# nikkolasg/playsnark

Measured on NVIDIA B200. Metric: g1_msm_points_per_s, higher is better.
Workload: dtype u32

## Files before the change

### playsnark_b200/build.py

```python
from __future__ import annotations

import glob
import os
import re
import subprocess
import sys
from concurrent.futures import ThreadPoolExecutor

HERE = os.path.dirname(os.path.abspath(__file__))
ROOT = os.path.dirname(HERE)
CSRC = os.path.join(HERE, "csrc")
OBJ = os.path.join(HERE, "_build")
LIB = os.path.join(HERE, "libplaysnark_b200.so")

CU_SOURCES = [os.path.join(CSRC, f) for f in ("capi.cu", "capi_poly.cu", "capi_multi.cu", "capi_verify.cu", "group_g1.cu", "group_g2.cu", "accum_g2.cu")
              if os.path.exists(os.path.join(CSRC, f))]

NVCC_FLAGS = [
    "-gencode", "arch=compute_100a,code=sm_100a", "-O3", "-std=c++17", "--expt-relaxed-constexpr",
    "-lineinfo", "-Xcompiler", "-fPIC",
]

_INC = re.compile(r'^\s*#\s*include\s+"([^"]+)"', re.M)


def _deps(path: str, seen=None):
    seen = set() if seen is None else seen
    path = os.path.normpath(path)
    if path in seen or not os.path.exists(path):
        return seen
    seen.add(path)
    with open(path) as f:
        for inc in _INC.findall(f.read()):
            _deps(os.path.join(os.path.dirname(path), inc), seen)
    return seen


def _sources():
    return sorted(glob.glob(os.path.join(CSRC, "*.cu")) + glob.glob(os.path.join(CSRC, "*.cuh")) +
                  [os.path.join(ROOT, "include", "playsnark_b200.h")])


def stale(target: str, sources) -> bool:
    if not os.path.exists(target):
        return True
    t = os.path.getmtime(target)
    return any(os.path.getmtime(s) > t for s in sources)


def build_cuda(force: bool = False, verbose: bool = False, out: str = LIB, extra_flags=()) -> str:
    if not force and not extra_flags and not stale(out, _sources()):
        return out
    nvcc = os.environ.get("NVCC", "nvcc")
    obj_dir = OBJ if out == LIB else out + ".obj"
    os.makedirs(obj_dir, exist_ok=True)
    jobs = []
    for src in CU_SOURCES:
        obj = os.path.join(obj_dir, os.path.basename(src)[:-3] + ".o")
        if force or extra_flags or stale(obj, _deps(src)):
            jobs.append((src, obj))
    threads = max(1, (os.cpu_count() or 2) // max(1, len(jobs)))

    def compile_one(job):
        src, obj = job
        cmd = [nvcc] + NVCC_FLAGS + list(extra_flags) + (["-Xptxas", "-v"] if verbose else []) + \
              ["-split-compile", str(threads), "-c", "-o", obj, src]
        print("[playsnark_b200] " + " ".join(cmd), file=sys.stderr)
        subprocess.check_call(cmd, cwd=ROOT)

    if jobs:
        with ThreadPoolExecutor(max_workers=len(jobs)) as ex:
            list(ex.map(compile_one, jobs))
    objs = [os.path.join(obj_dir, os.path.basename(s)[:-3] + ".o") for s in CU_SOURCES]
    cmd = [nvcc, "-gencode", "arch=compute_100a,code=sm_100a", "-shared", "-o", out] + objs
    print("[playsnark_b200] " + " ".join(cmd), file=sys.stderr)
    subprocess.check_call(cmd, cwd=ROOT)
    return out


def build_variant(name: str, flags, tus=("capi_poly.cu",)) -> str:
    build_cuda()
    nvcc = os.environ.get("NVCC", "nvcc")
    vdir = os.path.join(OBJ, "variants")
    os.makedirs(vdir, exist_ok=True)
    objs = []
    for src in CU_SOURCES:
        base = os.path.basename(src)
        if base in tus:
            obj = os.path.join(vdir, "%s_%s.o" % (base[:-3], name))
            if stale(obj, _deps(src)):
                cmd = [nvcc] + NVCC_FLAGS + list(flags) + ["-split-compile", "0", "-c", "-o", obj, src]
                print("[playsnark_b200] " + " ".join(cmd), file=sys.stderr)
                subprocess.check_call(cmd, cwd=ROOT)
        else:
            obj = os.path.join(OBJ, base[:-3] + ".o")
        objs.append(obj)
    os.makedirs(os.path.join(HERE, "variants"), exist_ok=True)
    out = os.path.join(HERE, "variants", "lib_%s.so" % name)
    subprocess.check_call([nvcc, "-gencode", "arch=compute_100a,code=sm_100a", "-shared", "-o", out] + objs, cwd=ROOT)
    return out


TEST_BUILD = os.path.join(ROOT, "tests", "_build")
DEVICE_HARNESS = os.path.join(ROOT, "tests", "device_arith.cu")


def can_write(dir_path: str) -> bool:
    while not os.path.isdir(dir_path):
        parent = os.path.dirname(dir_path)
        if parent == dir_path:
            return False
        dir_path = parent
    return os.access(dir_path, os.W_OK | os.X_OK)


def build_device_harness(out_dir: str = TEST_BUILD) -> str:
    so = os.path.join(out_dir, "libdevice_arith.so")
    if not stale(so, _deps(DEVICE_HARNESS)):
        return so
    os.makedirs(out_dir, exist_ok=True)
    tmp = "%s.%d.tmp" % (so, os.getpid())
    nvcc = os.environ.get("NVCC", "nvcc")
    cmd = [nvcc] + NVCC_FLAGS + ["-split-compile", "0", "-shared", "-o", tmp, DEVICE_HARNESS]
    print("[playsnark_b200] " + " ".join(cmd), file=sys.stderr)
    try:
        subprocess.check_call(cmd, cwd=ROOT)
        os.replace(tmp, so)
    finally:
        if os.path.exists(tmp):
            os.remove(tmp)
    return so


def build_host_emulation(out_dir: str) -> str:
    os.makedirs(out_dir, exist_ok=True)
    so = os.path.join(out_dir, "libps_hostemu.so")
    if not stale(so, _sources()):
        return so
    jobs = []
    for src in CU_SOURCES:
        obj = os.path.join(out_dir, "emu_" + os.path.basename(src)[:-3] + ".o")
        if stale(obj, _deps(src)):
            jobs.append((src, obj))

    def compile_one(job):
        src, obj = job
        subprocess.check_call(["g++", "-O2", "-std=c++17", "-x", "c++", "-DPS_HOST_EMU", "-fPIC", "-c", "-o", obj, src], cwd=ROOT)

    if jobs:
        with ThreadPoolExecutor(max_workers=len(jobs)) as ex:
            list(ex.map(compile_one, jobs))
    objs = [os.path.join(out_dir, "emu_" + os.path.basename(s)[:-3] + ".o") for s in CU_SOURCES]
    subprocess.check_call(["g++", "-shared", "-o", so] + objs + ["-lpthread"], cwd=ROOT)
    return so


if __name__ == "__main__":
    build_cuda(force="--force" in sys.argv, verbose="-v" in sys.argv)
```

### playsnark_b200/csrc/msm.cuh

```cuda
#pragma once
#include "group_ops.cuh"
#include "team.cuh"

namespace ps {

PS_DEV int msm_seg_of(const MsmPlan& p, uint32_t i) {
  int k = 0;
  while (k + 1 < p.nseg && i >= p.seg[k + 1].start) k++;
  return k;
}

PS_DEV void msm_load_scalar(const uint32_t* scalars, uint32_t i, int mont, uint32_t k[8], bool& neg) {
  Fr x;
#pragma unroll
  for (int j = 0; j < 8; j++) x.v[j] = scalars[(size_t)i * 8 + j];
  if (mont) x = x.from_mont();
  uint32_t t = ptx_sub_cc(FrParams::HALF(0), x.v[0]);
#pragma unroll
  for (int j = 1; j < 8; j++) t = ptx_subc_cc(FrParams::HALF(j), x.v[j]);
  uint32_t borrow = ptx_subc(0, 0);
  neg = borrow != 0;
  if (neg) {
    uint32_t m[8];
    m[0] = ptx_sub_cc(FrParams::MOD(0), x.v[0]);
#pragma unroll
    for (int j = 1; j < 8; j++) m[j] = ptx_subc_cc(FrParams::MOD(j), x.v[j]);
#pragma unroll
    for (int j = 0; j < 8; j++) x.v[j] = m[j];
  }
#pragma unroll
  for (int j = 0; j < 8; j++) k[j] = x.v[j];
}

PS_DEV uint32_t msm_take_bits(uint32_t k[8], int c) {
  uint32_t v = k[0] & ((1u << c) - 1);
#pragma unroll
  for (int j = 0; j < 7; j++) k[j] = (k[j] >> c) | (k[j + 1] << (32 - c));
  k[7] >>= c;
  return v;
}

PS_DEV bool msm_next_digit(uint32_t k[8], int c, uint32_t& carry, uint32_t& mag, bool& dneg) {
  uint32_t v = msm_take_bits(k, c) + carry;
  uint32_t half = 1u << (c - 1);
  if (v > half) { mag = (1u << c) - v; dneg = true; carry = 1; }
  else { mag = v; dneg = false; carry = 0; }
  return mag != 0;
}

struct MsmCountK {
  static constexpr int BLOCK = 256;
  PS_DEV static void run(uint32_t i, MsmPlan p, uint32_t* count, uint32_t* ranks) {
    const MsmSeg sg = p.seg[msm_seg_of(p, i)];
    uint32_t k[8]; bool neg;
    msm_load_scalar(sg.scalars, i - sg.start, (int)sg.mont, k, neg);
    uint32_t carry = 0;
    const uint32_t b0 = sg.set * (uint32_t)p.S * p.D;
    for (int w = 0; w < p.W; w++) {
      uint32_t mag; bool dneg;
      uint32_t rank = 0xFFFFFFFFu;
      if (msm_next_digit(k, p.c, carry, mag, dneg)) {
        uint32_t b = b0 + (uint32_t)(w / p.T) * p.D + (mag - 1);
        rank = ps_atomic_add(count + b, 1u);
      }
      ranks[(size_t)w * p.total + i] = rank;
    }
  }
};

struct MsmScatterK {
  static constexpr int BLOCK = 256;
  PS_DEV static void run(uint32_t i, MsmPlan p, const uint32_t* off, const uint32_t* ranks, uint32_t* ent) {
    const MsmSeg sg = p.seg[msm_seg_of(p, i)];
    uint32_t k[8]; bool neg;
    msm_load_scalar(sg.scalars, i - sg.start, (int)sg.mont, k, neg);
    uint32_t carry = 0;
    const uint32_t b0 = sg.set * (uint32_t)p.S * p.D, nbase = p.nbase[sg.set], pt = p.toff[sg.set] + sg.first + (i - sg.start);
    for (int w = 0; w < p.W; w++) {
      uint32_t mag; bool dneg;
      if (msm_next_digit(k, p.c, carry, mag, dneg)) {
        uint32_t b = b0 + (uint32_t)(w / p.T) * p.D + (mag - 1);
        uint32_t pos = off[b] + ranks[(size_t)w * p.total + i];
        uint32_t idx = (uint32_t)(w % p.T) * nbase + pt;
        ent[pos] = idx | ((neg != dneg) ? 0x80000000u : 0u);
      }
    }
  }
};

PS_DEV uint32_t msm_find_bucket(const uint32_t* off, uint32_t nb, uint32_t pos) {
  uint32_t lo = 0, hi = nb;
  while (hi - lo > 1) {
    uint32_t mid = lo + (hi - lo) / 2;
    if (off[mid] <= pos) lo = mid; else hi = mid;
  }
  return lo;
}

template <class F>
PS_DEV Affine<F> msm_load_point(const Affine<F>* tab, uint32_t e) {
  Affine<F> p = tab[e & 0x7FFFFFFFu];
  if (e >> 31) p.y = p.y.neg();
  return p;
}

#ifndef PS_G1_MINB
#define PS_G1_MINB 3
#endif
#ifndef PS_G2_MINB
#define PS_G2_MINB 2
#endif
#ifndef PS_ACC_BLOCK
#define PS_ACC_BLOCK 128
#endif
template <class F>
struct MsmAccumK {
  static constexpr int BLOCK = PS_ACC_BLOCK;
  static constexpr int MIN_BLOCKS = sizeof(F) == sizeof(Fp) ? PS_G1_MINB : PS_G2_MINB;
  using Self = MsmAccumK<F>;
  PS_DEV static void run(uint32_t tid, uint32_t nb, uint32_t L, const Affine<F>* tab, const uint32_t* ent,
                         const uint32_t* off, XYZZ<F>* buckets, XYZZ<F>* slot_pt, int32_t* slot_bid,
                         uint8_t* slot_fl) {
    const uint32_t M = off[nb];
    const uint32_t head = 2 * tid, tail = 2 * tid + 1;
    slot_bid[head] = -1; slot_bid[tail] = -1;
    uint64_t p0 = (uint64_t)tid * L;
    if (p0 >= M) return;
    uint32_t cur = (uint32_t)p0;
    uint32_t end = (M - cur > L) ? cur + L : M;
    uint32_t b = msm_find_bucket(off, nb, cur);
    bool head_open = off[b] < cur;
    uint32_t bend = off[b + 1];
    XYZZ<F> acc = XYZZ<F>::inf();
    for (; cur < end; cur++) {
      if (cur == bend) {
        flush(b, acc, head_open, true, head, tail, buckets, slot_pt, slot_bid, slot_fl);
        acc = XYZZ<F>::inf();
        head_open = false;
        b++;
        while (off[b + 1] <= cur) b++;
        bend = off[b + 1];
      }
      xyzz_madd(acc, msm_load_point(tab, ent[cur]));
    }
    flush(b, acc, head_open, bend <= end, head, tail, buckets, slot_pt, slot_bid, slot_fl);
  }
  PS_DEV static void flush(uint32_t b, const XYZZ<F>& acc, bool head_open, bool closed, uint32_t head, uint32_t tail,
                           XYZZ<F>* buckets, XYZZ<F>* slot_pt, int32_t* slot_bid, uint8_t* slot_fl) {
    if (closed && !head_open) {
      buckets[b] = acc;
    } else {
      uint32_t s = head_open ? head : tail;
      slot_pt[s] = acc;
      slot_bid[s] = (int32_t)b;
      slot_fl[s] = (uint8_t)((head_open ? 1 : 0) | (closed ? 0 : 2));
    }
  }
};

template <bool T> struct Coop;
template <> struct Coop<false> {
  static constexpr uint32_t LANES = 1;
  PS_DEV explicit Coop(uint32_t&) {}
  template <class F> PS_DEV void add(XYZZ<F>& acc, const XYZZ<F>& q) const { xyzz_add_c(acc, q); }
  template <class F> PS_DEV void dbl(XYZZ<F>& p) const { p = xyzz_dbl_c(p); }
  PS_DEV bool writer() const { return true; }
  PS_DEV bool idle() const { return false; }
  PS_DEV void sync() const {}
};
template <> struct Coop<true> {
  static constexpr uint32_t LANES = TEAM;
  TeamCtx tc;
  PS_DEV explicit Coop(uint32_t& tid) : tc(TeamCtx::of(tid)) { tid >>= 2; }
  template <class F> PS_DEV void add(XYZZ<F>& acc, const XYZZ<F>& q) const { xyzz_add_t(acc, q, tc); }
  template <class F> PS_DEV void dbl(XYZZ<F>& p) const { xyzz_dbl_t(p, tc); }
  PS_DEV bool writer() const { return tc.tl == 0; }
  PS_DEV bool idle() const {
#ifdef __CUDA_ARCH__
    return false;
#else
    return tc.tl != 0;
#endif
  }
  PS_DEV void sync() const { tc.sync(); }
};

template <class F, bool T>
struct MsmRunMergeK {
  static constexpr int BLOCK = 128;
  static constexpr uint32_t RUN_MAX = 32;
  PS_DEV static void run(uint32_t t, uint32_t n_chunks, XYZZ<F>* buckets, XYZZ<F>* slot_pt, int32_t* slot_bid,
                         const uint8_t* slot_fl) {
    Coop<T> co(t);
    if (co.idle()) return;
    const uint32_t a = 2 * t + 1;
    int32_t bid = slot_bid[a];
    if (bid < 0 || slot_fl[a] != 2) return;
    uint32_t len = 0;
    for (uint32_t j = 1; j <= RUN_MAX && t + j < n_chunks; j++) {
      uint32_t h = 2 * (t + j);
      if (slot_bid[h] != bid) return;
      if (slot_fl[h] == 1) { len = j; break; }
    }
    if (!len) return;
    XYZZ<F> acc = slot_pt[a];
    for (uint32_t j = 1; j <= len; j++) co.add(acc, slot_pt[2 * (t + j)]);
    co.sync();
    if (!co.writer()) return;
    buckets[bid] = acc;
    slot_bid[a] = -1;
    for (uint32_t j = 1; j <= len; j++) slot_bid[2 * (t + j)] = -1;
  }
};

template <class F, bool T>
struct MsmCombineK {
  static constexpr int BLOCK = 128;
  PS_DEV static void flush(int32_t bid, const XYZZ<F>& acc, bool cl, bool cr, int final_pass, uint32_t tid,
                           XYZZ<F>* buckets, XYZZ<F>* out_pt, int32_t* out_bid, uint8_t* out_fl) {
    if (bid < 0) return;
    if (final_pass || (!cl && !cr)) { buckets[bid] = acc; return; }
    uint32_t s = cl ? 2 * tid : 2 * tid + 1;
    out_pt[s] = acc; out_bid[s] = bid; out_fl[s] = (uint8_t)((cl ? 1 : 0) | (cr ? 2 : 0));
  }
  PS_DEV static void run(uint32_t tid, uint32_t n_in, uint32_t f, const XYZZ<F>* in_pt, const int32_t* in_bid,
                         const uint8_t* in_fl, XYZZ<F>* buckets, XYZZ<F>* out_pt, int32_t* out_bid,
                         uint8_t* out_fl, int final_pass) {
    Coop<T> co(tid);
    if (co.idle()) return;
    const bool wr = co.writer();
    if (wr) { out_bid[2 * tid] = -1; out_bid[2 * tid + 1] = -1; }
    int32_t cur = -1; bool cl = false, cr = false;
    XYZZ<F> acc = XYZZ<F>::inf();
    for (uint32_t i = 0; i < f; i++) {
      uint64_t j = (uint64_t)tid * f + i;
      if (j >= n_in) break;
      int32_t bid = in_bid[j];
      if (bid < 0) continue;
      uint8_t fl = in_fl[j];
      if (bid != cur) {
        if (wr) flush(cur, acc, cl, cr, final_pass, tid, buckets, out_pt, out_bid, out_fl);
        cur = bid; acc = in_pt[j]; cl = fl & 1; cr = (fl & 2) != 0;
      } else {
        co.add(acc, in_pt[j]); cr = (fl & 2) != 0;
      }
    }
    if (wr) flush(cur, acc, cl, cr, final_pass, tid, buckets, out_pt, out_bid, out_fl);
  }
};

template <class F, bool T>
struct MsmReduceFirstK {
  static constexpr int BLOCK = 128;
  PS_DEV static void run(uint32_t tid, uint32_t D, uint32_t G, uint32_t g, const XYZZ<F>* buckets, XYZZ<F>* acc_out,
                         XYZZ<F>* run_out) {
    Coop<T> co(tid);
    if (co.idle()) return;
    uint32_t s = tid / G, j = tid % G;
    const XYZZ<F>* B = buckets + (size_t)s * D + (size_t)j * g;
    XYZZ<F> rr = XYZZ<F>::inf(), ww = XYZZ<F>::inf();
    for (uint32_t i = g; i-- > 0;) {
      co.add(rr, B[i]);
      co.add(ww, rr);
    }
    if (co.writer()) { acc_out[tid] = ww; run_out[tid] = rr; }
  }
};

template <class F, bool T>
struct MsmReduceK {
  static constexpr int BLOCK = 64;
  PS_DEV static void run(uint32_t tid, uint32_t n_in, uint32_t n_out, uint32_t f, int log_len, const XYZZ<F>* acc_in,
                         const XYZZ<F>* run_in, XYZZ<F>* acc_out, XYZZ<F>* run_out) {
    Coop<T> co(tid);
    if (co.idle()) return;
    uint32_t s = tid / n_out, j = tid % n_out;
    const XYZZ<F>* A = acc_in + (size_t)s * n_in + (size_t)j * f;
    const XYZZ<F>* R = run_in + (size_t)s * n_in + (size_t)j * f;
    XYZZ<F> asum = XYZZ<F>::inf(), rr = XYZZ<F>::inf(), ww = XYZZ<F>::inf();
    for (uint32_t i = f; i-- > 0;) {
      if ((size_t)j * f + i >= n_in) continue;
      co.add(asum, A[i]);
      co.add(rr, R[i]);
      if (i > 0) co.add(ww, rr);
    }
    for (int d = 0; d < log_len; d++) co.dbl(ww);
    co.add(asum, ww);
    if (co.writer()) { acc_out[tid] = asum; run_out[tid] = rr; }
  }
};

template <class F, bool T>
struct MsmBitGatherK {
  static constexpr int BLOCK = 64;
  PS_DEV static void run(uint32_t tid, uint32_t G, int g, const XYZZ<F>* acc, const XYZZ<F>* run, XYZZ<F>* Y) {
    Coop<T> co(tid);
    if (co.idle()) return;
    const uint32_t half = G / 2;
    uint32_t s = tid / ((uint32_t)(g + 1) * half), rem = tid % ((uint32_t)(g + 1) * half);
    uint32_t r = rem / half, i = rem % half;
    XYZZ<F> y;
    if (r == 0) {
      y = acc[(size_t)s * G + 2 * i];
      co.add(y, acc[(size_t)s * G + 2 * i + 1]);
    } else {
      uint32_t k = r - 1;
      uint32_t j = ((i >> k) << (k + 1)) | (1u << k) | (i & ((1u << k) - 1));
      y = run[(size_t)s * G + j];
    }
    if (co.writer()) Y[tid] = y;
  }
};
template <class F, bool T>
struct MsmPairSumK {
  static constexpr int BLOCK = 64;
  PS_DEV static void run(uint32_t tid, uint32_t n_in, const XYZZ<F>* in, XYZZ<F>* out) {
    Coop<T> co(tid);
    if (co.idle()) return;
    uint32_t half = n_in / 2;
    uint32_t row = tid / half, i = tid % half;
    XYZZ<F> y = in[(size_t)row * n_in + 2 * i];
    co.add(y, in[(size_t)row * n_in + 2 * i + 1]);
    if (co.writer()) out[tid] = y;
  }
};
template <class F, bool T>
struct MsmBitFinalK {
  static constexpr int BLOCK = 32;
  PS_DEV static void run(uint32_t s, int g, int log_len, const XYZZ<F>* Y, XYZZ<F>* out) {
    Coop<T> co(s);
    if (co.idle()) return;
    const XYZZ<F>* row = Y + (size_t)s * (g + 1);
    XYZZ<F> r = XYZZ<F>::inf();
    for (int k = g - 1; k >= 0; k--) {
      co.dbl(r);
      co.add(r, row[k + 1]);
    }
    for (int d = 0; d < log_len; d++) co.dbl(r);
    co.add(r, row[0]);
    if (co.writer()) out[s] = r;
  }
};

template <class F, bool T>
struct MsmFinalK {
  static constexpr int BLOCK = 32;
  PS_DEV static void run(uint32_t tid, int S, int shift, const XYZZ<F>* sets, XYZZ<F>* out) {
    Coop<T> co(tid);
    if (co.idle()) return;
    XYZZ<F> r = XYZZ<F>::inf();
    for (int s = S - 1; s >= 0; s--) {
      for (int d = 0; d < shift; d++) co.dbl(r);
      co.add(r, sets[(size_t)tid * S + s]);
    }
    if (co.writer()) out[tid] = r;
  }
};

template <class F, bool T>
struct MsmSumK {
  static constexpr int BLOCK = 32;
  PS_DEV static void run(uint32_t tid, uint32_t count, const XYZZ<F>* in, XYZZ<F>* out) {
    Coop<T> co(tid);
    if (co.idle()) return;
    if (tid != 0) return;
    XYZZ<F> r = XYZZ<F>::inf();
    for (uint32_t i = 0; i < count; i++) co.add(r, in[i]);
    if (co.writer()) *out = r;
  }
};

#if PS_GPU
static constexpr int SCAN_THREADS = 256;
static constexpr int SCAN_ITEMS = 8;
static constexpr int SCAN_TILE = SCAN_THREADS * SCAN_ITEMS;

static __global__ void __launch_bounds__(SCAN_THREADS) k_scan_tiles(const uint32_t* in, uint32_t* out, uint32_t* tile_sums, uint32_t n) {
  __shared__ uint32_t warp_sums[SCAN_THREADS / 32];
  uint32_t base = blockIdx.x * SCAN_TILE + threadIdx.x * SCAN_ITEMS;
  uint32_t v[SCAN_ITEMS];
  uint32_t local = 0;
#pragma unroll
  for (int i = 0; i < SCAN_ITEMS; i++) { v[i] = (base + i < n) ? in[base + i] : 0; local += v[i]; }
  uint32_t lane = threadIdx.x & 31, wid = threadIdx.x >> 5;
  uint32_t inc = local;
#pragma unroll
  for (int d = 1; d < 32; d <<= 1) { uint32_t t = __shfl_up_sync(0xffffffffu, inc, d); if (lane >= d) inc += t; }
  if (lane == 31) warp_sums[wid] = inc;
  __syncthreads();
  if (wid == 0) {
    uint32_t ws = lane < SCAN_THREADS / 32 ? warp_sums[lane] : 0;
#pragma unroll
    for (int d = 1; d < 32; d <<= 1) { uint32_t t = __shfl_up_sync(0xffffffffu, ws, d); if (lane >= d) ws += t; }
    if (lane < SCAN_THREADS / 32) warp_sums[lane] = ws;
  }
  __syncthreads();
  uint32_t excl = inc - local + (wid ? warp_sums[wid - 1] : 0);
#pragma unroll
  for (int i = 0; i < SCAN_ITEMS; i++) { if (base + i < n) out[base + i] = excl; excl += v[i]; }
  if (threadIdx.x == SCAN_THREADS - 1) tile_sums[blockIdx.x] = warp_sums[SCAN_THREADS / 32 - 1];
}
static __global__ void __launch_bounds__(1024) k_scan_sums(uint32_t* sums, uint32_t n) {
  __shared__ uint32_t warp_sums[32];
  __shared__ uint32_t carry_s;
  if (threadIdx.x == 0) carry_s = 0;
  __syncthreads();
  uint32_t lane = threadIdx.x & 31, wid = threadIdx.x >> 5;
  for (uint32_t base = 0; base < n; base += 1024) {
    uint32_t idx = base + threadIdx.x;
    uint32_t v = idx < n ? sums[idx] : 0;
    uint32_t inc = v;
#pragma unroll
    for (int d = 1; d < 32; d <<= 1) { uint32_t t = __shfl_up_sync(0xffffffffu, inc, d); if (lane >= d) inc += t; }
    if (lane == 31) warp_sums[wid] = inc;
    __syncthreads();
    if (wid == 0) {
      uint32_t ws = warp_sums[lane];
#pragma unroll
      for (int d = 1; d < 32; d <<= 1) { uint32_t t = __shfl_up_sync(0xffffffffu, ws, d); if (lane >= d) ws += t; }
      warp_sums[lane] = ws;
    }
    __syncthreads();
    uint32_t carry = carry_s;
    uint32_t excl = carry + inc - v + (wid ? warp_sums[wid - 1] : 0);
    if (idx < n) sums[idx] = excl;
    __syncthreads();
    if (threadIdx.x == 1023) carry_s = carry + warp_sums[31];
    __syncthreads();
  }
}
static __global__ void __launch_bounds__(SCAN_THREADS) k_scan_add(uint32_t* out, const uint32_t* tile_sums, uint32_t n) {
  uint32_t base = blockIdx.x * SCAN_TILE + threadIdx.x * SCAN_ITEMS;
  uint32_t add = tile_sums[blockIdx.x];
#pragma unroll
  for (int i = 0; i < SCAN_ITEMS; i++) if (base + i < n) out[base + i] += add;
}
#endif

inline int exclusive_scan_u32(ps_stream_t st, const uint32_t* in, uint32_t* out, uint32_t* tile_sums, uint32_t n) {
#if PS_GPU
  uint32_t tiles = (n + SCAN_TILE - 1) / SCAN_TILE;
  k_scan_tiles<<<tiles, SCAN_THREADS, 0, st>>>(in, out, tile_sums, n);
  k_scan_sums<<<1, 1024, 0, st>>>(tile_sums, tiles);
  k_scan_add<<<tiles, SCAN_THREADS, 0, st>>>(out, tile_sums, n);
  PS_CUDA_TRY(cudaGetLastError());
  launch_counter() += 3;
#else
  (void)st; (void)tile_sums;
  uint32_t acc = 0;
  for (uint32_t i = 0; i < n; i++) { uint32_t v = in[i]; out[i] = acc; acc += v; }
#endif
  return PS_OK;
}

struct MsmStageScatterK {
  static constexpr int BLOCK = 256;
  PS_DEV static void run(uint32_t j, int shift, const uint32_t* part_count, const uint32_t* staging, uint32_t* ent) {
    const uint32_t part = j >> shift, k = j & ((1u << shift) - 1);
    if (k >= part_count[part]) return;
    const uint32_t pos = staging[2 * (size_t)j], val = staging[2 * (size_t)j + 1];
    ent[pos] = val;
  }
};
constexpr int SCATTER2_WMAX = 16;
#ifndef PS_SCATTER2_BLOCK
#define PS_SCATTER2_BLOCK 512
#endif
constexpr int SCATTER2_BLOCK = PS_SCATTER2_BLOCK;
#if PS_GPU
static __global__ void __launch_bounds__(SCATTER2_BLOCK) k_scatter_stage(MsmPlan p, const uint32_t* off, const uint32_t* ranks,
                                                             uint32_t* part_count, uint32_t* staging, int shift, uint32_t nparts) {
  extern __shared__ uint32_t sh_scatter[];
  uint32_t* hist = sh_scatter;
  uint32_t* base = sh_scatter + nparts;
  for (uint32_t q = threadIdx.x; q < nparts; q += blockDim.x) hist[q] = 0;
  __syncthreads();
  const uint32_t i = blockIdx.x * blockDim.x + threadIdx.x;
  uint32_t pos[SCATTER2_WMAX], val[SCATTER2_WMAX], lr[SCATTER2_WMAX];
#pragma unroll
  for (int w = 0; w < SCATTER2_WMAX; w++) pos[w] = 0xFFFFFFFFu;
  if (i < p.total) {
    const MsmSeg sg = p.seg[msm_seg_of(p, i)];
    uint32_t k[8]; bool neg;
    msm_load_scalar(sg.scalars, i - sg.start, (int)sg.mont, k, neg);
    uint32_t carry = 0;
    const uint32_t b0 = sg.set * (uint32_t)p.S * p.D, nbase = p.nbase[sg.set], pt = p.toff[sg.set] + sg.first + (i - sg.start);
#pragma unroll
    for (int w = 0; w < SCATTER2_WMAX; w++) {
      if (w < p.W) {
        uint32_t mag; bool dneg;
        if (msm_next_digit(k, p.c, carry, mag, dneg)) {
          const uint32_t b = b0 + (uint32_t)(w / p.T) * p.D + (mag - 1);
          pos[w] = off[b] + ranks[(size_t)w * p.total + i];
          val[w] = ((uint32_t)(w % p.T) * nbase + pt) | ((neg != dneg) ? 0x80000000u : 0u);
          lr[w] = atomicAdd(&hist[pos[w] >> shift], 1u);
        }
      }
    }
  }
  __syncthreads();
  for (uint32_t q = threadIdx.x; q < nparts; q += blockDim.x)
    if (hist[q]) base[q] = atomicAdd(&part_count[q], hist[q]);
  __syncthreads();
#pragma unroll
  for (int w = 0; w < SCATTER2_WMAX; w++) {
    if (pos[w] != 0xFFFFFFFFu) {
      const uint32_t part = pos[w] >> shift;
      const size_t slot = ((size_t)part << shift) + base[part] + lr[w];
      reinterpret_cast<uint2*>(staging)[slot] = make_uint2(pos[w], val[w]);
    }
  }
}
#endif
inline int scatter_stage(ps_stream_t st, const MsmPlan& p, const uint32_t* off, const uint32_t* ranks, uint32_t* part_count,
                         uint32_t* staging, int shift, uint32_t nparts) {
#if PS_GPU
  const uint32_t blocks = (p.total + SCATTER2_BLOCK - 1) / SCATTER2_BLOCK;
  k_scatter_stage<<<blocks, SCATTER2_BLOCK, 2 * nparts * sizeof(uint32_t), st>>>(p, off, ranks, part_count, staging, shift, nparts);
  PS_CUDA_TRY(cudaGetLastError());
  launch_counter()++;
#else
  (void)st; (void)nparts;
  for (uint32_t i = 0; i < p.total; i++) {
    const MsmSeg sg = p.seg[msm_seg_of(p, i)];
    uint32_t k[8]; bool neg;
    msm_load_scalar(sg.scalars, i - sg.start, (int)sg.mont, k, neg);
    uint32_t carry = 0;
    const uint32_t b0 = sg.set * (uint32_t)p.S * p.D, nbase = p.nbase[sg.set], pt = p.toff[sg.set] + sg.first + (i - sg.start);
    for (int w = 0; w < p.W; w++) {
      uint32_t mag; bool dneg;
      if (!msm_next_digit(k, p.c, carry, mag, dneg)) continue;
      const uint32_t b = b0 + (uint32_t)(w / p.T) * p.D + (mag - 1);
      const uint32_t pos = off[b] + ranks[(size_t)w * p.total + i];
      const uint32_t part = pos >> shift;
      const size_t slot = ((size_t)part << shift) + part_count[part]++;
      staging[2 * slot] = pos;
      staging[2 * slot + 1] = ((uint32_t)(w % p.T) * nbase + pt) | ((neg != dneg) ? 0x80000000u : 0u);
    }
  }
#endif
  return PS_OK;
}

template <class F>
inline int launch_accum(ps_stream_t st, size_t T1, uint32_t nb, uint32_t L, const Affine<F>* tab, const uint32_t* ent, const uint32_t* off,
                        XYZZ<F>* buckets, XYZZ<F>* slot_pt, int32_t* slot_bid, uint8_t* slot_fl) {
  PS_LAUNCH(MsmAccumK<F>, st, T1, nb, L, tab, ent, off, buckets, slot_pt, slot_bid, slot_fl);
  return PS_OK;
}
int launch_accum_g2(ps_stream_t st, size_t T1, uint32_t nb, uint32_t L, const Affine<Fp2>* tab, const uint32_t* ent, const uint32_t* off,
                    XYZZ<Fp2>* buckets, XYZZ<Fp2>* slot_pt, int32_t* slot_bid, uint8_t* slot_fl);
template <>
inline int launch_accum<Fp2>(ps_stream_t st, size_t T1, uint32_t nb, uint32_t L, const Affine<Fp2>* tab, const uint32_t* ent,
                             const uint32_t* off, XYZZ<Fp2>* buckets, XYZZ<Fp2>* slot_pt, int32_t* slot_bid, uint8_t* slot_fl) {
  return launch_accum_g2(st, T1, nb, L, tab, ent, off, buckets, slot_pt, slot_bid, slot_fl);
}

#ifndef PS_TEAM_MAX_ITEMS
#define PS_TEAM_MAX_ITEMS 65536
#endif
template <template <class, bool> class K, class F, class... Args>
inline int launch_coop(bool team, ps_stream_t st, size_t items, Args... args) {
  if (team && items <= PS_TEAM_MAX_ITEMS) return ps_launch<K<F, true>>(st, items * TEAM, args...);
  return ps_launch<K<F, false>>(st, items, args...);
}

template <class F>
int msm_run_batch(ps_ctx* ctx, const MsmPlan& g, const Affine<F>* tab, XYZZ<F>* d_out) {
  ps_stream_t st = ctx->stream;
  Arena& ar = ctx->arena;
  if (g.nsets < 1 || g.nsets > MSM_MAX_SEG || g.nseg < 0 || g.nseg > MSM_MAX_SEG) return PS_ERR_ARG;
  if (g.total == 0) return dev_memset(d_out, 0, (size_t)g.nsets * sizeof(XYZZ<F>), st);
  const int S_all = g.nsets * g.S;
  const uint32_t nb = (uint32_t)S_all * g.D;
  const size_t max_ent = (size_t)g.total * g.W;
  if (max_ent >= 0xFFFFFFFFull || (uint64_t)S_all * g.D >= 0x7FFFFFFFull) return PS_ERR_UNSUPPORTED;

  const size_t avg_bucket = max_ent / nb + 1;
  uint32_t L0 = 8;
  while (L0 < 512 && L0 < avg_bucket) L0 <<= 1;
  if (L0 < 512 && max_ent / (2 * (size_t)L0) >= 400000) L0 <<= 1;
  const size_t R = (size_t)ctx->sm_count * MsmAccumK<F>::MIN_BLOCKS * MsmAccumK<F>::BLOCK;
  size_t waves = (max_ent + R * L0 - 1) / (R * L0);
  if (ctx->msm_wave_floor && L0 <= 128 && waves > 1 && waves < 6) waves = max_ent / (R * L0);
  uint32_t L = waves >= 6 ? L0 : (uint32_t)((max_ent + waves * R - 1) / (waves * R));
  if (L < 8) L = 8;
  const size_t T1 = (max_ent + L - 1) / L;
  const uint32_t CF = 64;
  const bool team = ctx->msm_team != 0;

  uint32_t* count = ar.take<uint32_t>((size_t)nb + 1);
  uint32_t* off = ar.take<uint32_t>((size_t)nb + 1);
  uint32_t* tile_sums = ar.take<uint32_t>((size_t)nb / 2048 + 2);
  uint32_t* ranks = ar.take<uint32_t>(max_ent);
  uint32_t* ent = ar.take<uint32_t>(max_ent);
  XYZZ<F>* buckets = ar.take<XYZZ<F>>(nb);
  if (!count || !off || !tile_sums || !ranks || !ent || !buckets) return PS_ERR_ALLOC;

  ctx->ev_valid = false;
  PS_TRY(ctx_event(ctx, 0));
  PS_TRY(dev_memset(count, 0, ((size_t)nb + 1) * 4, st));
  PS_TRY(dev_memset(buckets, 0, (size_t)nb * sizeof(XYZZ<F>), st));
  PS_LAUNCH(MsmCountK, st, g.total, g, count, ranks);
  PS_TRY(exclusive_scan_u32(st, count, off, tile_sums, nb + 1));
  const bool two_pass = g.W <= SCATTER2_WMAX && (ctx->msm_scatter == 2 || (ctx->msm_scatter == 1 && max_ent >= ((size_t)1 << 27)));
  if (two_pass) {
    int shift = 20;
    while ((max_ent >> shift) >= 1024) shift++;
    const uint32_t nparts = (uint32_t)((max_ent + ((size_t)1 << shift) - 1) >> shift);
    uint32_t* part_count = ar.take<uint32_t>(nparts);
    uint32_t* staging = ar.take<uint32_t>(2 * ((size_t)nparts << shift));
    if (!part_count || !staging) return PS_ERR_ALLOC;
    PS_TRY(dev_memset(part_count, 0, (size_t)nparts * 4, st));
    PS_TRY(scatter_stage(st, g, off, ranks, part_count, staging, shift, nparts));
    PS_LAUNCH(MsmStageScatterK, st, (size_t)nparts << shift, shift, (const uint32_t*)part_count, (const uint32_t*)staging, ent);
  } else {
    PS_LAUNCH(MsmScatterK, st, g.total, g, (const uint32_t*)off, (const uint32_t*)ranks, ent);
  }
  PS_TRY(ctx_event(ctx, 1));
  {
    size_t slots_a = 2 * T1, slots_b = 2 * ((slots_a + CF - 1) / CF);
    XYZZ<F>* sp[2] = {ar.take<XYZZ<F>>(slots_a), ar.take<XYZZ<F>>(slots_b)};
    int32_t* sb[2] = {ar.take<int32_t>(slots_a), ar.take<int32_t>(slots_b)};
    uint8_t* sf[2] = {ar.take<uint8_t>(slots_a), ar.take<uint8_t>(slots_b)};
    if (!sp[0] || !sp[1] || !sb[0] || !sb[1] || !sf[0] || !sf[1]) return PS_ERR_ALLOC;
    PS_TRY((launch_accum<F>(st, T1, nb, L, tab, ent, off, buckets, sp[0], sb[0], sf[0])));
    PS_TRY(ctx_event(ctx, 2));
    PS_TRY((launch_coop<MsmRunMergeK, F>(team, st, T1, (uint32_t)T1, buckets, sp[0], sb[0], (const uint8_t*)sf[0])));
    {
      size_t n_in = slots_a;
      int cur = 0;
      for (;;) {
        size_t threads = (n_in + CF - 1) / CF;
        int final_pass = threads == 1;
        PS_TRY((launch_coop<MsmCombineK, F>(team, st, threads, (uint32_t)n_in, CF, (const XYZZ<F>*)sp[cur], (const int32_t*)sb[cur],
                                            (const uint8_t*)sf[cur], buckets, sp[cur ^ 1], sb[cur ^ 1], sf[cur ^ 1], final_pass)));
        if (final_pass) break;
        n_in = 2 * threads;
        cur ^= 1;
      }
    }
  }
  PS_TRY(ctx_event(ctx, 3));
  {
    uint32_t gsz = 1;
    while ((uint64_t)S_all * (g.D / gsz) > 131072 && gsz < g.D) gsz <<= 1;
    if (gsz < 2 && g.D >= 2) gsz = 2;
    if (gsz > g.D) gsz = g.D;
    uint32_t G = g.D / gsz;
    size_t e0 = (size_t)S_all * G;
    XYZZ<F>* accv[2] = {ar.take<XYZZ<F>>(e0), ar.take<XYZZ<F>>(e0 / 2 + S_all)};
    XYZZ<F>* runv[2] = {ar.take<XYZZ<F>>(e0), ar.take<XYZZ<F>>(e0 / 2 + S_all)};
    if (!accv[0] || !accv[1] || !runv[0] || !runv[1]) return PS_ERR_ALLOC;
    PS_TRY((launch_coop<MsmReduceFirstK, F>(team && e0 <= 32768, st, e0, g.D, G, gsz, (const XYZZ<F>*)buckets, accv[0], runv[0])));
    uint32_t n_in = G;
    int log_len = 0;
    while ((1u << log_len) < gsz) log_len++;
    int cur = 0;
    while (n_in > 8192) {
      uint32_t f = 4, n_out = n_in / f;
      PS_TRY((launch_coop<MsmReduceK, F>(team, st, (size_t)S_all * n_out, n_in, n_out, f, log_len, (const XYZZ<F>*)accv[cur],
                                         (const XYZZ<F>*)runv[cur], accv[cur ^ 1], runv[cur ^ 1])));
      log_len += 2;
      n_in = n_out;
      cur ^= 1;
    }
    XYZZ<F>* sets = accv[cur];
    if (n_in > 1) {
      int gb = 0;
      while ((1u << gb) < n_in) gb++;
      const uint32_t half = n_in / 2;
      size_t rows = (size_t)S_all * (gb + 1);
      XYZZ<F>* Y[2] = {ar.take<XYZZ<F>>(rows * half), ar.take<XYZZ<F>>(rows * (half / 2 + 1))};
      XYZZ<F>* set_out = ar.take<XYZZ<F>>(S_all);
      if (!Y[0] || !Y[1] || !set_out) return PS_ERR_ALLOC;
      PS_TRY((launch_coop<MsmBitGatherK, F>(team, st, rows * half, n_in, gb, (const XYZZ<F>*)accv[cur], (const XYZZ<F>*)runv[cur], Y[0])));
      int yc = 0;
      for (uint32_t w = half; w > 1; w >>= 1) {
        PS_TRY((launch_coop<MsmPairSumK, F>(team, st, rows * (w / 2), w, (const XYZZ<F>*)Y[yc], Y[yc ^ 1])));
        yc ^= 1;
      }
      PS_TRY((launch_coop<MsmBitFinalK, F>(team, st, (size_t)S_all, gb, log_len, (const XYZZ<F>*)Y[yc], set_out)));
      sets = set_out;
    }
    PS_TRY((launch_coop<MsmFinalK, F>(team, st, (size_t)g.nsets, g.S, g.c * g.T, (const XYZZ<F>*)sets, d_out)));
  }
  PS_TRY(ctx_event(ctx, 4));
  ctx->ev_valid = true;
  return PS_OK;
}

}
```

Measured before the change: 193.8 million.

## Replace two-pass MSM scatter with partitioned bucket-range sort and shrink run-merge length

Replaces the rank-based count/scatter path for large MSMs with a two-level partitioned sort. Scalars are first binned into coarse bucket-range partitions through shared-memory staging buffers, then each fixed-size tile is sorted into its final bucket positions using shared-memory histograms and warp-aggregated atomics. This is meant to cut the scattered global writes and drop the per-entry ranks array. The change also lowers RUN_MAX in the run-merge kernel from 32 to 8, which alters how merge work is split. In exchange it adds several extra kernel launches and scans, plus padded staging memory.

New measurement: 201.2 million (median of 6 runs). 3.8% higher.

```diff
diff --git a/playsnark_b200/build.py b/playsnark_b200/build.py
--- a/playsnark_b200/build.py
+++ b/playsnark_b200/build.py
@@ -132,25 +132,27 @@
     return so
 
 
-def build_host_emulation(out_dir: str) -> str:
+def build_host_emulation(out_dir: str, name: str = "", defines=()) -> str:
     os.makedirs(out_dir, exist_ok=True)
-    so = os.path.join(out_dir, "libps_hostemu.so")
+    tag = "emu_" + (name + "_" if name else "")
+    so = os.path.join(out_dir, "libps_hostemu%s.so" % ("_" + name if name else ""))
     if not stale(so, _sources()):
         return so
     jobs = []
     for src in CU_SOURCES:
-        obj = os.path.join(out_dir, "emu_" + os.path.basename(src)[:-3] + ".o")
+        obj = os.path.join(out_dir, tag + os.path.basename(src)[:-3] + ".o")
         if stale(obj, _deps(src)):
             jobs.append((src, obj))
 
     def compile_one(job):
         src, obj = job
-        subprocess.check_call(["g++", "-O2", "-std=c++17", "-x", "c++", "-DPS_HOST_EMU", "-fPIC", "-c", "-o", obj, src], cwd=ROOT)
+        subprocess.check_call(["g++", "-O2", "-std=c++17", "-x", "c++", "-DPS_HOST_EMU"] + ["-D" + d for d in defines] +
+                              ["-fPIC", "-c", "-o", obj, src], cwd=ROOT)
 
     if jobs:
         with ThreadPoolExecutor(max_workers=len(jobs)) as ex:
             list(ex.map(compile_one, jobs))
-    objs = [os.path.join(out_dir, "emu_" + os.path.basename(s)[:-3] + ".o") for s in CU_SOURCES]
+    objs = [os.path.join(out_dir, tag + os.path.basename(s)[:-3] + ".o") for s in CU_SOURCES]
     subprocess.check_call(["g++", "-shared", "-o", so] + objs + ["-lpthread"], cwd=ROOT)
     return so
 
diff --git a/playsnark_b200/csrc/msm.cuh b/playsnark_b200/csrc/msm.cuh
--- a/playsnark_b200/csrc/msm.cuh
+++ b/playsnark_b200/csrc/msm.cuh
@@ -1,4 +1,6 @@
 #pragma once
+#include <algorithm>
+
 #include "group_ops.cuh"
 #include "team.cuh"
 
@@ -185,10 +187,13 @@
   PS_DEV void sync() const { tc.sync(); }
 };
 
+#ifndef PS_RUN_MAX
+#define PS_RUN_MAX 8
+#endif
 template <class F, bool T>
 struct MsmRunMergeK {
   static constexpr int BLOCK = 128;
-  static constexpr uint32_t RUN_MAX = 32;
+  static constexpr uint32_t RUN_MAX = PS_RUN_MAX;
   PS_DEV static void run(uint32_t t, uint32_t n_chunks, XYZZ<F>* buckets, XYZZ<F>* slot_pt, int32_t* slot_bid,
                          const uint8_t* slot_fl) {
     Coop<T> co(t);
@@ -453,91 +458,263 @@
   return PS_OK;
 }
 
-struct MsmStageScatterK {
+#ifndef PS_SORT_TILE
+#define PS_SORT_TILE 32768
+#endif
+#ifndef PS_SORT_PARTS
+#define PS_SORT_PARTS 512
+#endif
+constexpr uint32_t SORT_TILE = PS_SORT_TILE;
+constexpr uint32_t SORT_PARTS = PS_SORT_PARTS;
+constexpr uint32_t SORT_SMEM_WORDS = 10240;
+constexpr uint32_t SORT_BUF_PAIRS = 12288;
+constexpr int SORT_BIN_BLOCK = 512;
+constexpr int SORT_BIN_PER_THREAD = 4;
+constexpr uint32_t SORT_BIN_SCALARS = SORT_BIN_BLOCK * SORT_BIN_PER_THREAD;
+constexpr int SORT_TILE_BLOCK = 512;
+
+struct alignas(8) MsmPair {
+  uint32_t b, e;
+};
+
+struct MsmSortGeom {
+  int shift;
+  uint32_t nparts;
+  size_t tiles;
+};
+inline uint32_t msm_sort_bin_scalars(int W) { return SORT_BUF_PAIRS / (uint32_t)W; }
+inline size_t msm_sort_bin_smem(uint32_t nparts) { return (size_t)SORT_BUF_PAIRS * 8 + 3 * (size_t)nparts * 4; }
+inline bool msm_sort_geom(uint32_t nb, size_t max_ent, MsmSortGeom& s) {
+  s.shift = 0;
+  while ((((uint64_t)nb + (1ull << s.shift) - 1) >> s.shift) > SORT_PARTS && (2u << s.shift) <= SORT_SMEM_WORDS) s.shift++;
+  s.nparts = (uint32_t)(((uint64_t)nb + (1ull << s.shift) - 1) >> s.shift);
+  s.tiles = (max_ent + SORT_TILE - 1) / SORT_TILE + s.nparts;
+  return s.nparts <= SORT_SMEM_WORDS && s.tiles * SORT_TILE < 0xFFFFFFFFull;
+}
+
+template <class Fn>
+PS_DEV void msm_digits(const MsmPlan& p, uint32_t i, Fn f) {
+  const MsmSeg sg = p.seg[msm_seg_of(p, i)];
+  uint32_t k[8]; bool neg;
+  msm_load_scalar(sg.scalars, i - sg.start, (int)sg.mont, k, neg);
+  uint32_t carry = 0;
+  const uint32_t b0 = sg.set * (uint32_t)p.S * p.D, nbase = p.nbase[sg.set], pt = p.toff[sg.set] + sg.first + (i - sg.start);
+  for (int w = 0; w < p.W; w++) {
+    uint32_t mag; bool dneg;
+    if (msm_next_digit(k, p.c, carry, mag, dneg))
+      f(b0 + (uint32_t)(w / p.T) * p.D + (mag - 1), ((uint32_t)(w % p.T) * nbase + pt) | ((neg != dneg) ? 0x80000000u : 0u));
+  }
+}
+
+struct MsmSortPadK {
   static constexpr int BLOCK = 256;
-  PS_DEV static void run(uint32_t j, int shift, const uint32_t* part_count, const uint32_t* staging, uint32_t* ent) {
-    const uint32_t part = j >> shift, k = j & ((1u << shift) - 1);
-    if (k >= part_count[part]) return;
-    const uint32_t pos = staging[2 * (size_t)j], val = staging[2 * (size_t)j + 1];
-    ent[pos] = val;
-  }
-};
-constexpr int SCATTER2_WMAX = 16;
-#ifndef PS_SCATTER2_BLOCK
-#define PS_SCATTER2_BLOCK 512
-#endif
-constexpr int SCATTER2_BLOCK = PS_SCATTER2_BLOCK;
+  PS_DEV static void run(uint32_t q, const uint32_t* pcnt, uint32_t* padded) {
+    padded[q] = (pcnt[q] + SORT_TILE - 1) / SORT_TILE * SORT_TILE;
+  }
+};
+
 #if PS_GPU
-static __global__ void __launch_bounds__(SCATTER2_BLOCK) k_scatter_stage(MsmPlan p, const uint32_t* off, const uint32_t* ranks,
-                                                             uint32_t* part_count, uint32_t* staging, int shift, uint32_t nparts) {
-  extern __shared__ uint32_t sh_scatter[];
-  uint32_t* hist = sh_scatter;
-  uint32_t* base = sh_scatter + nparts;
-  for (uint32_t q = threadIdx.x; q < nparts; q += blockDim.x) hist[q] = 0;
-  __syncthreads();
-  const uint32_t i = blockIdx.x * blockDim.x + threadIdx.x;
-  uint32_t pos[SCATTER2_WMAX], val[SCATTER2_WMAX], lr[SCATTER2_WMAX];
-#pragma unroll
-  for (int w = 0; w < SCATTER2_WMAX; w++) pos[w] = 0xFFFFFFFFu;
-  if (i < p.total) {
-    const MsmSeg sg = p.seg[msm_seg_of(p, i)];
-    uint32_t k[8]; bool neg;
-    msm_load_scalar(sg.scalars, i - sg.start, (int)sg.mont, k, neg);
-    uint32_t carry = 0;
-    const uint32_t b0 = sg.set * (uint32_t)p.S * p.D, nbase = p.nbase[sg.set], pt = p.toff[sg.set] + sg.first + (i - sg.start);
-#pragma unroll
-    for (int w = 0; w < SCATTER2_WMAX; w++) {
-      if (w < p.W) {
+static __device__ __forceinline__ uint32_t sort_inc(uint32_t* h, uint32_t key, bool live) {
+  const uint32_t act = __ballot_sync(0xFFFFFFFFu, live);
+  if (!act) return 0;
+  const int lead = __ffs(act) - 1;
+  const uint32_t k0 = __shfl_sync(0xFFFFFFFFu, key, lead);
+  if (__ballot_sync(0xFFFFFFFFu, live && key == k0) == act) {
+    const uint32_t lane = threadIdx.x & 31;
+    uint32_t base = 0;
+    if ((int)lane == lead) base = atomicAdd(&h[k0], (uint32_t)__popc(act));
+    base = __shfl_sync(0xFFFFFFFFu, base, lead);
+    return base + (uint32_t)__popc(act & ((1u << lane) - 1));
+  }
+  return live ? atomicAdd(&h[key], 1u) : 0;
+}
+
+static __device__ uint32_t sort_block_scan(const uint32_t* a, uint32_t* out, uint32_t n) {
+  __shared__ uint32_t ws[SORT_BIN_BLOCK / 32];
+  const uint32_t per = (n + SORT_BIN_BLOCK - 1) / SORT_BIN_BLOCK;
+  const uint32_t lo = min(n, threadIdx.x * per), hi = min(n, lo + per);
+  uint32_t sum = 0;
+  for (uint32_t x = lo; x < hi; x++) sum += a[x];
+  const uint32_t lane = threadIdx.x & 31, wid = threadIdx.x >> 5;
+  uint32_t inc = sum;
+#pragma unroll
+  for (int d = 1; d < 32; d <<= 1) { const uint32_t t = __shfl_up_sync(0xFFFFFFFFu, inc, d); if (lane >= (uint32_t)d) inc += t; }
+  if (lane == 31) ws[wid] = inc;
+  __syncthreads();
+  if (wid == 0) {
+    uint32_t v = lane < SORT_BIN_BLOCK / 32 ? ws[lane] : 0;
+#pragma unroll
+    for (int d = 1; d < 32; d <<= 1) { const uint32_t t = __shfl_up_sync(0xFFFFFFFFu, v, d); if (lane >= (uint32_t)d) v += t; }
+    if (lane < SORT_BIN_BLOCK / 32) ws[lane] = v;
+  }
+  __syncthreads();
+  uint32_t run = inc - sum + (wid ? ws[wid - 1] : 0);
+  for (uint32_t x = lo; x < hi; x++) { out[x] = run; run += a[x]; }
+  return ws[SORT_BIN_BLOCK / 32 - 1];
+}
+
+template <bool COUNT>
+static __global__ void __launch_bounds__(SORT_BIN_BLOCK) k_sort_bin(MsmPlan p, uint32_t spb, int shift, uint32_t nparts, uint32_t* pcnt,
+                                                                    uint32_t* pcur, const uint32_t* pst, MsmPair* staging) {
+  extern __shared__ uint2 sh_bin[];
+  MsmPair* buf = reinterpret_cast<MsmPair*>(sh_bin);
+  uint32_t* cnt = reinterpret_cast<uint32_t*>(sh_bin) + (COUNT ? 0 : 2 * SORT_BUF_PAIRS);
+  uint32_t* lst = cnt + nparts;
+  uint32_t* gb = lst + nparts;
+  for (uint32_t q = threadIdx.x; q < nparts; q += SORT_BIN_BLOCK) cnt[q] = 0;
+  __syncthreads();
+  const uint32_t i0 = blockIdx.x * spb, i1 = min(p.total, i0 + spb);
+  auto pass = [&](bool place) {
+    for (uint32_t j = 0; j < spb; j += SORT_BIN_BLOCK) {
+      const uint32_t i = i0 + j + threadIdx.x;
+      const bool in = i < i1;
+      const MsmSeg sg = p.seg[in ? msm_seg_of(p, i) : 0];
+      uint32_t k[8] = {0, 0, 0, 0, 0, 0, 0, 0}; bool neg = false;
+      if (in) msm_load_scalar(sg.scalars, i - sg.start, (int)sg.mont, k, neg);
+      uint32_t carry = 0;
+      const uint32_t b0 = sg.set * (uint32_t)p.S * p.D, nbase = p.nbase[sg.set], pt = p.toff[sg.set] + sg.first + (i - sg.start);
+      for (int w = 0; w < p.W; w++) {
         uint32_t mag; bool dneg;
-        if (msm_next_digit(k, p.c, carry, mag, dneg)) {
-          const uint32_t b = b0 + (uint32_t)(w / p.T) * p.D + (mag - 1);
-          pos[w] = off[b] + ranks[(size_t)w * p.total + i];
-          val[w] = ((uint32_t)(w % p.T) * nbase + pt) | ((neg != dneg) ? 0x80000000u : 0u);
-          lr[w] = atomicAdd(&hist[pos[w] >> shift], 1u);
-        }
+        const bool live = msm_next_digit(k, p.c, carry, mag, dneg) && in;
+        const uint32_t b = b0 + (uint32_t)(w / p.T) * p.D + (mag - 1);
+        const uint32_t r = sort_inc(cnt, b >> shift, live);
+        if (place && live) buf[r] = MsmPair{b, ((uint32_t)(w % p.T) * nbase + pt) | ((neg != dneg) ? 0x80000000u : 0u)};
       }
     }
-  }
-  __syncthreads();
-  for (uint32_t q = threadIdx.x; q < nparts; q += blockDim.x)
-    if (hist[q]) base[q] = atomicAdd(&part_count[q], hist[q]);
-  __syncthreads();
-#pragma unroll
-  for (int w = 0; w < SCATTER2_WMAX; w++) {
-    if (pos[w] != 0xFFFFFFFFu) {
-      const uint32_t part = pos[w] >> shift;
-      const size_t slot = ((size_t)part << shift) + base[part] + lr[w];
-      reinterpret_cast<uint2*>(staging)[slot] = make_uint2(pos[w], val[w]);
-    }
-  }
-}
-#endif
-inline int scatter_stage(ps_stream_t st, const MsmPlan& p, const uint32_t* off, const uint32_t* ranks, uint32_t* part_count,
-                         uint32_t* staging, int shift, uint32_t nparts) {
+  };
+  pass(false);
+  __syncthreads();
+  if (COUNT) {
+    for (uint32_t q = threadIdx.x; q < nparts; q += SORT_BIN_BLOCK)
+      if (cnt[q]) atomicAdd(&pcnt[q], cnt[q]);
+    return;
+  }
+  const uint32_t npairs = sort_block_scan(cnt, lst, nparts);
+  __syncthreads();
+  for (uint32_t q = threadIdx.x; q < nparts; q += SORT_BIN_BLOCK) {
+    if (cnt[q]) gb[q] = pst[q] + atomicAdd(&pcur[q], cnt[q]);
+    cnt[q] = lst[q];
+  }
+  __syncthreads();
+  pass(true);
+  __syncthreads();
+  for (uint32_t x = threadIdx.x; x < npairs; x += SORT_BIN_BLOCK) {
+    const MsmPair pr = buf[x];
+    const uint32_t q = pr.b >> shift;
+    staging[gb[q] + (x - lst[q])] = pr;
+  }
+}
+
+template <bool COUNT>
+static __global__ void __launch_bounds__(SORT_TILE_BLOCK) k_sort_tile(uint32_t nb, int shift, uint32_t nparts, const uint32_t* pcnt,
+                                                                      const uint32_t* pst, const MsmPair* staging, uint32_t* count,
+                                                                      const uint32_t* off, uint32_t* cursor, uint32_t* ent) {
+  extern __shared__ uint32_t sh_sort[];
+  const uint32_t start = blockIdx.x * SORT_TILE;
+  if (start >= pst[nparts]) return;
+  const uint32_t q = msm_find_bucket(pst, nparts, start);
+  const uint32_t n = min(SORT_TILE, pst[q] + pcnt[q] - start);
+  const uint32_t base = q << shift, nbk = min(1u << shift, nb - base);
+  for (uint32_t x = threadIdx.x; x < nbk; x += SORT_TILE_BLOCK) sh_sort[x] = 0;
+  __syncthreads();
+  const uint32_t nr = (n + SORT_TILE_BLOCK - 1) / SORT_TILE_BLOCK * SORT_TILE_BLOCK;
+  for (uint32_t e = threadIdx.x; e < nr; e += SORT_TILE_BLOCK)
+    sort_inc(sh_sort, e < n ? staging[start + e].b - base : 0, e < n);
+  __syncthreads();
+  for (uint32_t x = threadIdx.x; x < nbk; x += SORT_TILE_BLOCK) {
+    const uint32_t h = sh_sort[x];
+    if (!h) continue;
+    if (COUNT) atomicAdd(&count[base + x], h);
+    else sh_sort[x] = off[base + x] + atomicAdd(&cursor[base + x], h);
+  }
+  if (COUNT) return;
+  __syncthreads();
+  for (uint32_t e = threadIdx.x; e < nr; e += SORT_TILE_BLOCK) {
+    const MsmPair pr = e < n ? staging[start + e] : MsmPair{base, 0};
+    const uint32_t r = sort_inc(sh_sort, pr.b - base, e < n);
+    if (e < n) ent[r] = pr.e;
+  }
+}
+#endif
+
+inline int msm_sort_partitioned(ps_ctx* ctx, const MsmPlan& p, const MsmSortGeom& sg, uint32_t nb, uint32_t* count, uint32_t* off, uint32_t* tile_sums, uint32_t* ent) {
+  ps_stream_t st = ctx->stream;
+  Arena& ar = ctx->arena;
+  const uint32_t np = sg.nparts;
+  uint32_t* pw = ar.take<uint32_t>(3 * ((size_t)np + 1));
+  uint32_t* pst = ar.take<uint32_t>((size_t)np + 1);
+  uint32_t* stg = ar.take<uint32_t>(2 * sg.tiles * SORT_TILE);
+  uint32_t* tsum = ar.take<uint32_t>((size_t)np / 2048 + 2);
+  if (!pw || !pst || !stg || !tsum) return PS_ERR_ALLOC;
+  uint32_t *pcnt = pw, *pcur = pw + np + 1, *padded = pw + 2 * ((size_t)np + 1);
+  MsmPair* staging = reinterpret_cast<MsmPair*>(stg);
+  PS_TRY(dev_memset(pw, 0, 2 * ((size_t)np + 1) * 4, st));
 #if PS_GPU
-  const uint32_t blocks = (p.total + SCATTER2_BLOCK - 1) / SCATTER2_BLOCK;
-  k_scatter_stage<<<blocks, SCATTER2_BLOCK, 2 * nparts * sizeof(uint32_t), st>>>(p, off, ranks, part_count, staging, shift, nparts);
+  const uint32_t spb = msm_sort_bin_scalars(p.W);
+  const uint32_t counts = (p.total + SORT_BIN_SCALARS - 1) / SORT_BIN_SCALARS, bins = (p.total + spb - 1) / spb;
+  const size_t bin_smem = msm_sort_bin_smem(np), tile_smem = ((size_t)1 << sg.shift) * 4;
+  PS_CUDA_TRY(cudaFuncSetAttribute(k_sort_bin<false>, cudaFuncAttributeMaxDynamicSharedMemorySize, (int)bin_smem));
+  k_sort_bin<true><<<counts, SORT_BIN_BLOCK, (size_t)np * 4, st>>>(p, SORT_BIN_SCALARS, sg.shift, np, pcnt, pcur, pst, staging);
   PS_CUDA_TRY(cudaGetLastError());
-  launch_counter()++;
+  PS_LAUNCH(MsmSortPadK, st, (size_t)np + 1, (const uint32_t*)pcnt, padded);
+  PS_TRY(exclusive_scan_u32(st, padded, pst, tsum, np + 1));
+  k_sort_bin<false><<<bins, SORT_BIN_BLOCK, bin_smem, st>>>(p, spb, sg.shift, np, pcnt, pcur, pst, staging);
+  PS_CUDA_TRY(cudaGetLastError());
+  k_sort_tile<true><<<(uint32_t)sg.tiles, SORT_TILE_BLOCK, tile_smem, st>>>(nb, sg.shift, np, pcnt, pst, staging, count, off, count, ent);
+  PS_CUDA_TRY(cudaGetLastError());
+  PS_TRY(exclusive_scan_u32(st, count, off, tile_sums, nb + 1));
+  PS_TRY(dev_memset(count, 0, (size_t)nb * 4, st));
+  k_sort_tile<false><<<(uint32_t)sg.tiles, SORT_TILE_BLOCK, tile_smem, st>>>(nb, sg.shift, np, pcnt, pst, staging, count, off, count, ent);
+  PS_CUDA_TRY(cudaGetLastError());
+  launch_counter() += 4;
 #else
-  (void)st; (void)nparts;
-  for (uint32_t i = 0; i < p.total; i++) {
-    const MsmSeg sg = p.seg[msm_seg_of(p, i)];
-    uint32_t k[8]; bool neg;
-    msm_load_scalar(sg.scalars, i - sg.start, (int)sg.mont, k, neg);
-    uint32_t carry = 0;
-    const uint32_t b0 = sg.set * (uint32_t)p.S * p.D, nbase = p.nbase[sg.set], pt = p.toff[sg.set] + sg.first + (i - sg.start);
-    for (int w = 0; w < p.W; w++) {
-      uint32_t mag; bool dneg;
-      if (!msm_next_digit(k, p.c, carry, mag, dneg)) continue;
-      const uint32_t b = b0 + (uint32_t)(w / p.T) * p.D + (mag - 1);
-      const uint32_t pos = off[b] + ranks[(size_t)w * p.total + i];
-      const uint32_t part = pos >> shift;
-      const size_t slot = ((size_t)part << shift) + part_count[part]++;
-      staging[2 * slot] = pos;
-      staging[2 * slot + 1] = ((uint32_t)(w % p.T) * nbase + pt) | ((neg != dneg) ? 0x80000000u : 0u);
-    }
-  }
+  std::vector<uint32_t> h(np);
+  auto bin = [&](bool place) {
+    const uint32_t spb = place ? msm_sort_bin_scalars(p.W) : SORT_BIN_SCALARS;
+    for (uint32_t i0 = 0; i0 < p.total; i0 += spb) {
+      const uint32_t i1 = p.total - i0 < spb ? p.total : i0 + spb;
+      std::fill(h.begin(), h.end(), 0u);
+      for (uint32_t i = i0; i < i1; i++) msm_digits(p, i, [&](uint32_t b, uint32_t) { h[b >> sg.shift]++; });
+      for (uint32_t q = 0; q < np; q++) {
+        if (!h[q]) continue;
+        if (!place) { pcnt[q] += h[q]; continue; }
+        const uint32_t r = pst[q] + pcur[q];
+        pcur[q] += h[q];
+        h[q] = r;
+      }
+      if (place)
+        for (uint32_t i = i0; i < i1; i++) msm_digits(p, i, [&](uint32_t b, uint32_t e) { staging[h[b >> sg.shift]++] = {b, e}; });
+    }
+  };
+  auto tiles = [&](bool place) {
+    std::vector<uint32_t> t((size_t)1 << sg.shift);
+    for (size_t x = 0; x < sg.tiles; x++) {
+      const uint32_t start = (uint32_t)(x * SORT_TILE);
+      if (start >= pst[np]) break;
+      const uint32_t q = msm_find_bucket(pst, np, start);
+      const uint32_t n = std::min(SORT_TILE, pst[q] + pcnt[q] - start);
+      const uint32_t base = q << sg.shift, nbk = std::min(1u << sg.shift, nb - base);
+      std::fill(t.begin(), t.end(), 0u);
+      for (uint32_t e = 0; e < n; e++) t[staging[start + e].b - base]++;
+      for (uint32_t b = 0; b < nbk; b++) {
+        if (!t[b]) continue;
+        if (!place) { count[base + b] += t[b]; continue; }
+        const uint32_t r = off[base + b] + count[base + b];
+        count[base + b] += t[b];
+        t[b] = r;
+      }
+      if (place)
+        for (uint32_t e = 0; e < n; e++) ent[t[staging[start + e].b - base]++] = staging[start + e].e;
+    }
+  };
+  bin(false);
+  PS_LAUNCH(MsmSortPadK, st, (size_t)np + 1, (const uint32_t*)pcnt, padded);
+  PS_TRY(exclusive_scan_u32(st, padded, pst, tsum, np + 1));
+  bin(true);
+  tiles(false);
+  PS_TRY(exclusive_scan_u32(st, count, off, tile_sums, nb + 1));
+  PS_TRY(dev_memset(count, 0, (size_t)nb * 4, st));
+  tiles(true);
 #endif
   return PS_OK;
 }
@@ -589,32 +766,29 @@
   const uint32_t CF = 64;
   const bool team = ctx->msm_team != 0;
 
+  MsmSortGeom sgeo;
+  const bool geo_ok = msm_sort_geom(nb, max_ent, sgeo);
+  if (ctx->msm_scatter == 2 && !geo_ok) return PS_ERR_UNSUPPORTED;
+  const bool partitioned = geo_ok && (ctx->msm_scatter == 2 || (ctx->msm_scatter == 1 && max_ent >= ((size_t)1 << 27)));
+
   uint32_t* count = ar.take<uint32_t>((size_t)nb + 1);
   uint32_t* off = ar.take<uint32_t>((size_t)nb + 1);
   uint32_t* tile_sums = ar.take<uint32_t>((size_t)nb / 2048 + 2);
-  uint32_t* ranks = ar.take<uint32_t>(max_ent);
   uint32_t* ent = ar.take<uint32_t>(max_ent);
   XYZZ<F>* buckets = ar.take<XYZZ<F>>(nb);
-  if (!count || !off || !tile_sums || !ranks || !ent || !buckets) return PS_ERR_ALLOC;
+  if (!count || !off || !tile_sums || !ent || !buckets) return PS_ERR_ALLOC;
 
   ctx->ev_valid = false;
   PS_TRY(ctx_event(ctx, 0));
   PS_TRY(dev_memset(count, 0, ((size_t)nb + 1) * 4, st));
   PS_TRY(dev_memset(buckets, 0, (size_t)nb * sizeof(XYZZ<F>), st));
-  PS_LAUNCH(MsmCountK, st, g.total, g, count, ranks);
-  PS_TRY(exclusive_scan_u32(st, count, off, tile_sums, nb + 1));
-  const bool two_pass = g.W <= SCATTER2_WMAX && (ctx->msm_scatter == 2 || (ctx->msm_scatter == 1 && max_ent >= ((size_t)1 << 27)));
-  if (two_pass) {
-    int shift = 20;
-    while ((max_ent >> shift) >= 1024) shift++;
-    const uint32_t nparts = (uint32_t)((max_ent + ((size_t)1 << shift) - 1) >> shift);
-    uint32_t* part_count = ar.take<uint32_t>(nparts);
-    uint32_t* staging = ar.take<uint32_t>(2 * ((size_t)nparts << shift));
-    if (!part_count || !staging) return PS_ERR_ALLOC;
-    PS_TRY(dev_memset(part_count, 0, (size_t)nparts * 4, st));
-    PS_TRY(scatter_stage(st, g, off, ranks, part_count, staging, shift, nparts));
-    PS_LAUNCH(MsmStageScatterK, st, (size_t)nparts << shift, shift, (const uint32_t*)part_count, (const uint32_t*)staging, ent);
+  if (partitioned) {
+    PS_TRY(msm_sort_partitioned(ctx, g, sgeo, nb, count, off, tile_sums, ent));
   } else {
+    uint32_t* ranks = ar.take<uint32_t>(max_ent);
+    if (!ranks) return PS_ERR_ALLOC;
+    PS_LAUNCH(MsmCountK, st, g.total, g, count, ranks);
+    PS_TRY(exclusive_scan_u32(st, count, off, tile_sums, nb + 1));
     PS_LAUNCH(MsmScatterK, st, g.total, g, (const uint32_t*)off, (const uint32_t*)ranks, ent);
   }
   PS_TRY(ctx_event(ctx, 1));
```
